# uthree/tinyvc

Hardware: AMD Instinct MI355X
Metric: audio-samples/sec (16 kHz) end-to-end VC (higher is better)
Workload: dtype f32 (fp32 in / out / accumulate; channel contractions as two-term fp16 splits on v_mfma_f32_32x32x16_f16: 22-bit significands, three part-products per fp32 product)

## Files before the change

### tinyvc_amd/csrc/knn.hip

```cpp
#include "knn_blob.h"
#include "knn_search.h"
#include "split_fp16.h"
#include "tvc_common.h"

namespace tvc {

constexpr int KNN_BLOCKS = 1024;

constexpr int QN_WAVES = 16;
static __global__ __launch_bounds__(QN_WAVES * 64) void query_normalize_kernel(const float* __restrict__ src, float* __restrict__ qn, int B, int Bsrc, int T,
                                                                     uint4* __restrict__ qh, int* __restrict__ cnt, int* __restrict__ flag,
                                                                     const KnnSegs segs, int* __restrict__ col2seg) {
    __shared__ float part[QN_WAVES][64];
    const int lane = threadIdx.x & 63, wave = threadIdx.x >> 6;
    const long ncols = (long)B * T;
    long n, nn;
    bool ok;
    int sg;
    if (qh) {
        const int tile = blockIdx.x >> 2;
        sg = seg_find<3>(segs, tile);
        const KnnSeg g = seg_get(segs, sg);
        const long loc = (long)(tile - g.u[3]) * 256 + (blockIdx.x & 3) * 64 + lane;
        ok = loc < g.ncols;
        n = g.col0 + loc;
        nn = ok ? n : g.col0 + g.ncols - 1;
    } else {
        n = blockIdx.x * 64L + lane;
        ok = n < ncols;
        nn = ok ? n : ncols - 1;
        sg = col2seg ? seg_find<4>(segs, (int)nn) : 0;
    }
    if (blockIdx.x == 0 && flag)
        for (int i = threadIdx.x; i < segs.n; i += QN_WAVES * 64) flag[i] = 0;
    if (wave == 0 && ok && cnt) cnt[n] = 0;
    if (wave == 0 && ok && col2seg) col2seg[n] = sg;
    const int b = (int)(nn / T), t = (int)(nn - (long)b * T);
    const float* p = src + (long)(b % Bsrc) * KD * T + t;
    float* q = qn + (long)b * KD * T + t;
    constexpr int KW = KD / QN_WAVES;
    const int k0 = wave * KW;
    float x[KW];
#pragma unroll
    for (int i = 0; i < KW; ++i) x[i] = p[(long)(k0 + i) * T];
    float s = 0.f;
#pragma unroll
    for (int i = 0; i < KW; ++i) s = fmaf(x[i], x[i], s);
    part[wave][lane] = s;
    __syncthreads();
    float ss = part[0][lane];
#pragma unroll
    for (int w = 1; w < QN_WAVES; ++w) ss += part[w][lane];
    const float den = sqrtf(ss) + 1e-6f;
    uint4* qhp = qh ? qh + (blockIdx.x >> 2) * (long)(STEPS * 2 * 256) + (blockIdx.x & 3) * 64 + lane : nullptr;
#pragma unroll
    for (int i = 0; i < KW; i += 8) {
        const int k = k0 + i;
        float v[8];
#pragma unroll
        for (int j = 0; j < 8; ++j) v[j] = ok ? x[i + j] / den : 0.f;
        if (ok) {
#pragma unroll
            for (int j = 0; j < 8; ++j) q[(long)(k + j) * T] = v[j];
        }
        if (qh) {
            unsigned o[4];
#pragma unroll
            for (int j = 0; j < 4; ++j) {
                const __half2 h = __floats2half2_rn(v[2 * j], v[2 * j + 1]);
                o[j] = (unsigned)__half_as_ushort(__low2half(h)) | ((unsigned)__half_as_ushort(__high2half(h)) << 16);
            }
            qhp[(long)(k >> 3) * 256] = make_uint4(o[0], o[1], o[2], o[3]);
        }
    }
}

typedef __bf16 bf16x8 __attribute__((ext_vector_type(8)));
typedef __bf16 bf16x2 __attribute__((ext_vector_type(2)));
__device__ __forceinline__ void split8_bf3(const float (&v)[8], uint4& p1, uint4& p2, uint4& p3) {
    unsigned o1[4], o2[4], o3[4];
#pragma unroll
    for (int j = 0; j < 4; ++j) {
        f32x2 a = {v[2 * j], v[2 * j + 1]};
        bf16x2 h1 = __builtin_convertvector(a, bf16x2);
        f32x2 r = a - __builtin_convertvector(h1, f32x2);
        bf16x2 h2 = __builtin_convertvector(r, bf16x2);
        f32x2 r2 = r - __builtin_convertvector(h2, f32x2);
        bf16x2 h3 = __builtin_convertvector(r2, bf16x2);
        o1[j] = __builtin_bit_cast(unsigned, h1);
        o2[j] = __builtin_bit_cast(unsigned, h2);
        o3[j] = __builtin_bit_cast(unsigned, h3);
    }
    p1 = make_uint4(o1[0], o1[1], o1[2], o1[3]);
    p2 = make_uint4(o2[0], o2[1], o2[2], o2[3]);
    p3 = make_uint4(o3[0], o3[1], o3[2], o3[3]);
}
__device__ __forceinline__ void split8_half(const u32x4 h8, uint4& p1, uint4& p2) {
    const f16x8 hv = __builtin_bit_cast(f16x8, h8);
    unsigned o1[4], o2[4];
#pragma unroll
    for (int j = 0; j < 4; ++j) {
        f32x2 a = {(float)hv[2 * j], (float)hv[2 * j + 1]};
        bf16x2 h1 = __builtin_convertvector(a, bf16x2);
        f32x2 r = a - __builtin_convertvector(h1, f32x2);
        bf16x2 h2 = __builtin_convertvector(r, bf16x2);
        o1[j] = __builtin_bit_cast(unsigned, h1);
        o2[j] = __builtin_bit_cast(unsigned, h2);
    }
    p1 = make_uint4(o1[0], o1[1], o1[2], o1[3]);
    p2 = make_uint4(o2[0], o2[1], o2[2], o2[3]);
}

constexpr int KNN_QT = 256;
constexpr int KNN_A_U4 = 12 * 64, KNN_X_U4 = 3 * 2 * KNN_QT;
template <bool F16>
__device__ __forceinline__ void knn_topk_body(const float* __restrict__ blob, long Npad, int N, const float* __restrict__ qn, int ncols, int col0, int cstride,
                                              int T, int unit, int nsplit, int tiles_per_split, float* __restrict__ cand_v, int* __restrict__ cand_i,
                                              uint4* smem) {
    constexpr int NP = F16 ? 2 : 3;
    constexpr int GP = F16 ? 4 : 12;
    uint4* As = smem;
    uint4* Xs = smem + 2 * KNN_A_U4;
    const uint4* img = F16 ? blob_img16(blob, KIND_F16, N, Npad) : blob_img3(blob, N);
    const float* inv = blob_inv(blob, KIND_F16, N, Npad);

    const int tid = threadIdx.x, lane = tid & 63, wave = tid >> 6;
    const int wm = wave >> 2, wn = wave & 3;
    const int l31 = lane & 31, lh = lane >> 5;
    const int split = unit % nsplit;
    const int qtile = unit / nsplit;
    const int n0 = qtile * KNN_QT;
    const int mtiles = (int)(Npad >> 7);
    const int mt_lo = split * tiles_per_split;
    const int mt_hi = min(mtiles, mt_lo + tiles_per_split);
    const int G = (mt_hi - mt_lo) * STEPS;

    const float* qp;
    int xdst;
    {
        const int g = tid >> 8, pos = tid & 255;
        int n = n0 + pos;
        n = col0 + (n < ncols ? n : ncols - 1);
        const int b = n / T, t = n - b * T;
        qp = qn + ((long)b * KD + 8 * g) * T + t;
        xdst = g * KNN_QT + pos;
    }
    const bool a2 = !F16 && wave < 4;
    const bool a1 = !F16 || wave < 4;
    float xr[8];
    u32x4 ar[2];
    auto gload = [&](int g) __attribute__((always_inline)) {
        const int mt = mt_lo + g / STEPS, st = g - (g / STEPS) * STEPS;
        const uint4* src = img + ((long)mt * STEPS + st) * (GP * 64) + lane;
        if (a1) ar[0] = *reinterpret_cast<const u32x4*>(src + wave * 64);
        if (a2) ar[1] = *reinterpret_cast<const u32x4*>(src + (wave + 8) * 64);
#pragma unroll
        for (int j = 0; j < 8; ++j) xr[j] = qp[(long)(st * 16 + j) * T];
    };
    auto lstore = [&](int buf) __attribute__((always_inline)) {
        uint4* ab = As + buf * KNN_A_U4;
        if (F16) {
            if (a1) {
                uint4 p1, p2;
                split8_half(ar[0], p1, p2);
                ab[(wave * 2) * 64 + lane] = p1;
                ab[(wave * 2 + 1) * 64 + lane] = p2;
            }
        } else {
            *reinterpret_cast<u32x4*>(ab + wave * 64 + lane) = ar[0];
            if (a2) *reinterpret_cast<u32x4*>(ab + (wave + 8) * 64 + lane) = ar[1];
        }
        uint4 p1, p2, p3;
        split8_bf3(xr, p1, p2, p3);
        uint4* xb = Xs + buf * KNN_X_U4;
        xb[xdst] = p1;
        xb[2 * KNN_QT + xdst] = p2;
        xb[4 * KNN_QT + xdst] = p3;
    };

    Top4 top[2];
    top[0].init();
    top[1].init();
    f32x16 acc[2][2];
#pragma unroll
    for (int i = 0; i < 2; ++i)
#pragma unroll
        for (int j = 0; j < 2; ++j)
#pragma unroll
            for (int r = 0; r < 16; ++r) acc[i][j][r] = 0.f;

    if (G > 0) {
        gload(0);
        lstore(0);
        if (G > 1) gload(1);
        slab_barrier();
    }
    for (int g = 0; g < G; ++g) {
        const int cur = g & 1;
        if (g + 1 < G) {
            lstore(cur ^ 1);
            if (g + 2 < G) gload(g + 2);
        }
        const uint4* as = As + cur * KNN_A_U4 + wm * (2 * NP * 64) + lane;
        const uint4* xs = Xs + cur * KNN_X_U4 + lh * KNN_QT + wn * 64 + l31;
        bf16x8 af[2][NP], bf[2][3];
#pragma unroll
        for (int j = 0; j < 2; ++j)
#pragma unroll
            for (int p = 0; p < 3; ++p) bf[j][p] = __builtin_bit_cast(bf16x8, xs[p * 2 * KNN_QT + j * 32]);
#pragma unroll
        for (int i = 0; i < 2; ++i)
#pragma unroll
            for (int p = 0; p < NP; ++p) af[i][p] = __builtin_bit_cast(bf16x8, as[(i * NP + p) * 64]);
        constexpr int NQ = F16 ? 5 : 6;
        constexpr int PA3[6] = {2, 1, 0, 1, 0, 0}, PB3[6] = {0, 1, 2, 0, 1, 0};
        constexpr int PA2[5] = {1, 0, 1, 0, 0}, PB2[5] = {1, 2, 0, 1, 0};
#pragma unroll
        for (int q = 0; q < NQ; ++q)
#pragma unroll
            for (int i = 0; i < 2; ++i)
#pragma unroll
                for (int j = 0; j < 2; ++j)
                    acc[i][j] = __builtin_amdgcn_mfma_f32_32x32x16_bf16(af[i][F16 ? PA2[q < 5 ? q : 0] : PA3[q]], bf[j][F16 ? PB2[q < 5 ? q : 0] : PB3[q]],
                                                                        acc[i][j], 0, 0, 0);
        const int st = g - (g / STEPS) * STEPS;
        if (st == STEPS - 1) {
            const int m0 = (mt_lo + g / STEPS) * 128;
#pragma unroll
            for (int i = 0; i < 2; ++i)
#pragma unroll
                for (int r = 0; r < 16; ++r) {
                    const int row = m0 + (wm * 2 + i) * 32 + (r & 3) + 8 * (r >> 2) + 4 * lh;
                    if (row < N) {
                        const float sc = F16 ? inv[row] : 1.f;
#pragma unroll
                        for (int j = 0; j < 2; ++j) top[j].insert(nan_max(F16 ? acc[i][j][r] * sc : acc[i][j][r]), row);
                    }
#pragma unroll
                    for (int j = 0; j < 2; ++j) acc[i][j][r] = 0.f;
                }
        }
        slab_barrier();
    }

    float (*mv)[16] = reinterpret_cast<float (*)[16]>(smem);
    int (*mi)[16] = reinterpret_cast<int (*)[16]>(reinterpret_cast<float*>(smem) + KNN_QT * 16);
#pragma unroll
    for (int j = 0; j < 2; ++j) {
        const int q = wn * 64 + j * 32 + l31;
        const int slot = (wm * 2 + lh) * 4;
#pragma unroll
        for (int e = 0; e < 4; ++e) {
            mv[q][slot + e] = top[j].v[e];
            mi[q][slot + e] = top[j].i[e];
        }
    }
    __syncthreads();
    if (tid < KNN_QT) {
        Top4 t4;
        t4.init();
        for (int e = 0; e < 16; ++e) t4.insert(mv[tid][e], mi[tid][e]);
        int n = n0 + tid;
        if (n < ncols) {
            long o = ((long)split * cstride + col0 + n) * 4;
#pragma unroll
            for (int e = 0; e < 4; ++e) {
                cand_v[o + e] = t4.v[e];
                cand_i[o + e] = t4.i[e];
            }
        }
    }
}

static __global__ __launch_bounds__(512) void knn_topk_split_kernel(const KnnSegs segs, const float* __restrict__ qn, int cstride, int T,
                                                                    float* __restrict__ cand_v, int* __restrict__ cand_i,
                                                                    const int* __restrict__ flags) {
    __shared__ __attribute__((aligned(16))) uint4 smem[2 * (KNN_A_U4 + KNN_X_U4)];
    const int si = seg_find<2>(segs, blockIdx.x);
    const KnnSeg g = seg_get(segs, si);
    if (g.two && flags[si] == 0) return;
    const int kind = blob_kind(g.blob);
    const int unit = blockIdx.x - g.u[2];
    if (kind == KIND_F16) knn_topk_body<true>(g.blob, blob_npad(g.N), g.N, qn, g.ncols, g.col0, cstride, T, unit, g.nsE, g.tpsE, cand_v, cand_i, smem);
    else knn_topk_body<false>(g.blob, blob_npad(g.N), g.N, qn, g.ncols, g.col0, cstride, T, unit, g.nsE, g.tpsE, cand_v, cand_i, smem);
}

constexpr int C_QT = 256, C_MT = 256, C_K = 64, C_STEPS = KD / C_K;
constexpr int C_A_U4 = 4 * 8 * 64, C_X_U4 = 4 * 2 * C_QT;
constexpr int C_LDS = 2 * (C_A_U4 + C_X_U4) * 16;
constexpr int C_CAP = 256;
constexpr float C_EPS = 1.25e-3f;
constexpr int KNN_COARSE_MIN = 4096;

struct Top4V {
    float v[4];
    __device__ __forceinline__ void init() { v[0] = v[1] = v[2] = v[3] = -INFINITY; }
    __device__ __forceinline__ void insert(float x) {
        if (!(x > v[3])) return;
        if (x > v[0]) { v[3] = v[2]; v[2] = v[1]; v[1] = v[0]; v[0] = x; }
        else if (x > v[1]) { v[3] = v[2]; v[2] = v[1]; v[1] = x; }
        else if (x > v[2]) { v[3] = v[2]; v[2] = x; }
        else v[3] = x;
    }
};

template <bool F16, int MODE>
static __device__ __forceinline__ void knn_coarse_body(const float* __restrict__ blob, long Npad, int N, const uint4* __restrict__ qh,
                                                       int ncols, int cstride, int unit, int nsplit, int tiles_per_split, int t2_cover,
                                                       float* __restrict__ c4v, int ns_sample,
                                                       int* __restrict__ cnt, int* __restrict__ cand, float* __restrict__ candv,
                                                       int* __restrict__ overflow) {
    extern __shared__ __attribute__((aligned(16))) uint4 csmem[];
    uint4* As = csmem;
    uint4* Xs = csmem + 2 * C_A_U4;
    const int kind = F16 ? KIND_F16 : KIND_F32;
    const uint4* img = blob_img16(blob, kind, N, Npad);
    const float* inv = blob_inv(blob, kind, N, Npad);

    const int tid = threadIdx.x, lane = tid & 63, wave = tid >> 6;
    const int wm = wave >> 2, wn = wave & 3;
    const int l31 = lane & 31, lh = lane >> 5;
    const int split = unit % nsplit;
    const int qtile = unit / nsplit;
    const int n0 = qtile * C_QT;
    const int mtiles = (int)(Npad >> 7);
    const int t_lo = split * tiles_per_split;
    const int t_hi = min(t2_cover, t_lo + tiles_per_split);
    const int G = (t_hi - t_lo) * C_STEPS;

    const uint4* xsrc = qh + (long)qtile * (STEPS * 2 * 256) + (tid & 511);
    u32x4 ar[4], xr[4];
    auto gload = [&](int g) __attribute__((always_inline)) {
        const int t2 = t_lo + g / C_STEPS, st = g - (g / C_STEPS) * C_STEPS;
#pragma unroll
        for (int i = 0; i < 4; ++i) {
            const int piece = wave + 8 * i, k16 = piece >> 3, mt8 = piece & 7;
            int t128 = 2 * t2 + (mt8 >> 2);
            t128 = t128 < mtiles ? t128 : mtiles - 1;
            ar[i] = *reinterpret_cast<const u32x4*>(img + (((long)t128 * STEPS + 4 * st + k16) * 4 + (mt8 & 3)) * 64 + lane);
            xr[i] = *reinterpret_cast<const u32x4*>(xsrc + (long)(4 * st + i) * 512);
        }
    };
    auto lstore = [&](int buf) __attribute__((always_inline)) {
#pragma unroll
        for (int i = 0; i < 4; ++i) {
            *reinterpret_cast<u32x4*>(As + buf * C_A_U4 + tid + 512 * i) = ar[i];
            *reinterpret_cast<u32x4*>(Xs + buf * C_X_U4 + tid + 512 * i) = xr[i];
        }
    };

    Top4V top[2];
    top[0].init();
    top[1].init();
    float th[2] = {INFINITY, INFINITY};
    if (MODE == 1) {
#pragma unroll
        for (int j = 0; j < 2; ++j) {
            const int n = n0 + wn * 64 + j * 32 + l31;
            if (n < ncols) {
                Top4V t4;
                t4.init();
                for (int sp = 0; sp < ns_sample; ++sp) {
                    const float4 v4 = *reinterpret_cast<const float4*>(c4v + ((long)sp * cstride + n) * 4);
                    t4.insert(v4.x);
                    t4.insert(v4.y);
                    t4.insert(v4.z);
                    t4.insert(v4.w);
// ... 64 lines not shown
                            const int row = m0 + (wm * 4 + i) * 32 + (r & 3) + 8 * (r >> 2) + 4 * lh;
                            if (whole || row < N) {
                                const float a = acc[i][j][r];
                                if (MODE == 0) {
                                    if (!F16) {
                                        top[j].insert(nan_max(a));
                                    } else if (!(fmaxf(a, 0.f) * imx <= top[j].v[3])) {
                                        top[j].insert(nan_max(a * inv[row]));
                                    }
                                } else {
                                    bool hit;
                                    float cv = a;
                                    if (!F16) hit = !(a < th[j]);
                                    else {
                                        hit = a != a || (fmaxf(a, 0.f) * imx >= th[j]);
                                        if (hit) {
                                            cv = a * inv[row];
                                            hit = a != a || cv >= th[j];
                                        }
                                    }
                                    hit = hit && th[j] != INFINITY;
                                    if (hit) {
                                        const int n = n0 + wn * 64 + j * 32 + l31;
                                        const int pos = atomicAdd(&cnt[n], 1);
                                        if (pos < C_CAP) {
                                            cand[(long)n * C_CAP + pos] = row;
                                            candv[(long)n * C_CAP + pos] = cv;
                                        } else *overflow = 1;
                                    }
                                }
                            }
                        }
                    }
#pragma unroll
                    for (int r = 0; r < 16; ++r) acc[i][j][r] = 0.f;
                }
        }
        slab_barrier();
    }
    if (MODE == 1) return;

    float (*mv)[16] = reinterpret_cast<float (*)[16]>(csmem);
#pragma unroll
    for (int j = 0; j < 2; ++j) {
        const int q = wn * 64 + j * 32 + l31;
        const int slot = (wm * 2 + lh) * 4;
#pragma unroll
        for (int e = 0; e < 4; ++e) mv[q][slot + e] = top[j].v[e];
    }
    __syncthreads();
    if (tid < C_QT) {
        Top4V t4;
        t4.init();
        for (int e = 0; e < 16; ++e) t4.insert(mv[tid][e]);
        const int n = n0 + tid;
        if (n < ncols) {
            const long o = ((long)split * cstride + n) * 4;
#pragma unroll
            for (int e = 0; e < 4; ++e) c4v[o + e] = t4.v[e];
        }
    }
}

template <int MODE>
static __global__ __launch_bounds__(512) void knn_coarse_kernel(const KnnSegs segs, const uint4* __restrict__ qh, int cstride,
                                                                float* __restrict__ c4v, int* __restrict__ cnt, int* __restrict__ cand,
                                                                float* __restrict__ candv, int* __restrict__ flags) {
    const int si = seg_find<MODE>(segs, blockIdx.x);
    const KnnSeg g = seg_get(segs, si);
    const int unit = blockIdx.x - g.u[MODE];
    const int nsplit = MODE ? g.nsB : g.nsA, tps = MODE ? g.tpsB : g.tpsA, cover = MODE ? g.t2 : g.sample;
    const uint4* q = qh + (long)g.u[3] * (STEPS * 2 * 256);
    float* c4 = c4v + (long)g.col0 * 4;
    int* ct = cnt + g.col0;
    int* cd = cand + (long)g.col0 * C_CAP;
    float* cdv = candv + (long)g.col0 * C_CAP;
    if (blob_kind(g.blob) == KIND_F16)
        knn_coarse_body<true, MODE>(g.blob, blob_npad(g.N), g.N, q, g.ncols, cstride, unit, nsplit, tps, cover, c4, g.nsA, ct, cd, cdv, flags + si);
    else
        knn_coarse_body<false, MODE>(g.blob, blob_npad(g.N), g.N, q, g.ncols, cstride, unit, nsplit, tps, cover, c4, g.nsA, ct, cd, cdv, flags + si);
}

static __global__ __launch_bounds__(256) void knn_rescore_kernel(const KnnSegs segs, const int* __restrict__ col2seg, const float* __restrict__ qn,
                                                                 int ncols, int T, const int* __restrict__ cnt, const int* __restrict__ cand,
                                                                 const float* __restrict__ candv, float* __restrict__ rv, int* __restrict__ ri) {
    constexpr int RG = 4;
    const int lane = threadIdx.x & 63;
    const int n = blockIdx.x * 4 + (threadIdx.x >> 6);
    if (n >= ncols) return;
    const KnnSeg g = seg_get(segs, col2seg ? __builtin_amdgcn_readfirstlane(col2seg[n]) : 0);
    if (!g.two) return;
    const float* __restrict__ blob = g.blob;
    const int N = g.N;
    const long Npad = blob_npad(g.N);
    const int kind = blob_kind(blob);
    const float* inv = blob_inv(blob, kind, N, Npad);
    const int b = n / T, t = n - b * T;
    const float* qp = qn + (long)b * KD * T + t;
    int rowl[C_CAP / 64];
    float cvl[C_CAP / 64];
#pragma unroll
    for (int c = 0; c < C_CAP / 64; ++c) {
        rowl[c] = cand[(long)n * C_CAP + 64 * c + lane];
        cvl[c] = candv[(long)n * C_CAP + 64 * c + lane];
    }
    const int nc = min(cnt[n], C_CAP);
    Top4 t4;
    t4.init();
    float th2;
    {
        float rk[C_CAP / 64];
#pragma unroll
        for (int c = 0; c < C_CAP / 64; ++c) {
            if (!(64 * c + lane < nc)) {
                cvl[c] = -INFINITY;
                rowl[c] = 0;
            }
            rk[c] = cvl[c] == cvl[c] ? cvl[c] : -INFINITY;
        }
        float wm = -INFINITY;
#pragma unroll
        for (int round = 0; round < 4; ++round) {
            float lm = rk[0];
#pragma unroll
            for (int c = 1; c < C_CAP / 64; ++c) lm = fmaxf(lm, rk[c]);
            wm = lm;
#pragma unroll
            for (int o = 32; o > 0; o >>= 1) wm = fmaxf(wm, __shfl_xor(wm, o));
            const unsigned long long who = __builtin_amdgcn_ballot_w64(lm == wm);
            if (lane == __builtin_ctzll(who)) {
                bool done = false;
#pragma unroll
                for (int c = 0; c < C_CAP / 64; ++c)
                    if (!done && rk[c] == wm) {
                        rk[c] = -INFINITY;
                        done = true;
                    }
            }
        }
        th2 = wm - 2.f * C_EPS;
    }
    static_assert(C_CAP == 256, "four 64-entry chunks");
    if (kind == KIND_F16) {
        const uint4* img = blob_img16(blob, kind, N, Npad);
        float qs[2][8];
#pragma unroll
        for (int h = 0; h < 2; ++h)
#pragma unroll
            for (int j = 0; j < 8; ++j) {
                const int seg = lane + 64 * h;
                qs[h][j] = seg < 96 ? qp[(long)(8 * seg + j) * T] : 0.f;
            }
        for (int base = 0, ch = 0; base < nc; base += 64, ++ch) {
            const int mine = ch == 0 ? rowl[0] : (ch == 1 ? rowl[1] : (ch == 2 ? rowl[2] : rowl[3]));
            const float cvv = ch == 0 ? cvl[0] : (ch == 1 ? cvl[1] : (ch == 2 ? cvl[2] : cvl[3]));
            unsigned long long mask = __builtin_amdgcn_ballot_w64(base + lane < nc && !(cvv < th2));
            while (mask) {
                int row[RG];
                bool live[RG];
                float d[RG], iv[RG];
                u32x4 w[RG][2];
                int pos = 0;
#pragma unroll
                for (int g = 0; g < RG; ++g) {
                    live[g] = mask != 0ull;
                    if (live[g]) {
                        pos = __builtin_ctzll(mask);
                        mask &= mask - 1;
                    }
                    row[g] = __shfl(mine, pos);
                    const long rbase = ((long)(row[g] >> 7) * STEPS * 4 + ((row[g] & 127) >> 5)) * 64 + (row[g] & 31);
#pragma unroll
                    for (int h = 0; h < 2; ++h) {
                        const int seg = lane + 64 * h < 96 ? lane + 64 * h : 0;
                        w[g][h] = *reinterpret_cast<const u32x4*>(img + rbase + (long)(seg >> 1) * 256 + (seg & 1) * 32);
                    }
                    iv[g] = inv[row[g]];
                }
#pragma unroll
                for (int g = 0; g < RG; ++g) {
                    d[g] = 0.f;
#pragma unroll
                    for (int h = 0; h < 2; ++h) {
                        if (lane + 64 * h < 96) {
                            const f16x8 hv = __builtin_bit_cast(f16x8, w[g][h]);
#pragma unroll
                            for (int j = 0; j < 8; ++j) d[g] = fmaf(qs[h][j], (float)hv[j], d[g]);
                        }
                    }
                }
#pragma unroll
                for (int o = 32; o > 0; o >>= 1)
#pragma unroll
                    for (int g = 0; g < RG; ++g) d[g] += __shfl_xor(d[g], o);
#pragma unroll
                for (int g = 0; g < RG; ++g)
                    if (live[g]) t4.insert(nan_max(d[g] * iv[g]), row[g]);
            }
        }
    } else {
        float qv[12];
#pragma unroll
        for (int u = 0; u < 12; ++u) qv[u] = qp[(long)(lane + 64 * u) * T];
        const float* rows = blob_rows(blob);
        for (int base = 0, ch = 0; base < nc; base += 64, ++ch) {
            const int mine = ch == 0 ? rowl[0] : (ch == 1 ? rowl[1] : (ch == 2 ? rowl[2] : rowl[3]));
            const float cvv = ch == 0 ? cvl[0] : (ch == 1 ? cvl[1] : (ch == 2 ? cvl[2] : cvl[3]));
            unsigned long long mask = __builtin_amdgcn_ballot_w64(base + lane < nc && !(cvv < th2));
            while (mask) {
                int row[RG];
                bool live[RG];
                float d[RG], iv[RG], xv[RG][12];
                int pos = 0;
#pragma unroll
                for (int g = 0; g < RG; ++g) {
                    live[g] = mask != 0ull;
                    if (live[g]) {
                        pos = __builtin_ctzll(mask);
                        mask &= mask - 1;
                    }
                    row[g] = __shfl(mine, pos);
                    const float* rp = rows + (long)row[g] * KD + lane;
#pragma unroll
                    for (int u = 0; u < 12; ++u) xv[g][u] = rp[64 * u];
                    iv[g] = inv[row[g]];
                }
#pragma unroll
                for (int g = 0; g < RG; ++g) {
                    d[g] = 0.f;
#pragma unroll
                    for (int u = 0; u < 12; ++u) d[g] = fmaf(qv[u], xv[g][u], d[g]);
                }
#pragma unroll
                for (int o = 32; o > 0; o >>= 1)
#pragma unroll
                    for (int g = 0; g < RG; ++g) d[g] += __shfl_xor(d[g], o);
#pragma unroll
                for (int g = 0; g < RG; ++g)
                    if (live[g]) t4.insert(nan_max(d[g] * iv[g]), row[g]);
            }
        }
    }
    if (nc < 4) {
#pragma unroll
        for (int e = 0; e < 4; ++e) {
            t4.v[e] = INFINITY;
            t4.i[e] = e;
        }
    }
    if (lane == 0) {
#pragma unroll
        for (int e = 0; e < 4; ++e) {
            rv[(long)n * 4 + e] = t4.v[e];
            ri[(long)n * 4 + e] = t4.i[e];
        }
    }
}

static void split_plan(int blocks, int qtiles, int cover, int* ns, int* tps) {
    int n = (blocks + qtiles - 1) / qtiles;
    if (n > cover) n = cover;
    if (n < 1) n = 1;
    *tps = (cover + n - 1) / n;
    *ns = (cover + *tps - 1) / *tps;
}

int knn_call_plan(tvc_ctx* ctx, const KnnSegIn* in, int nin, int ncols, KnnCall* c) {
    static_assert(KNN_QT == C_QT, "one query tiling for both searches");
    c->ncols = ncols;
    for (int i = 0; i < nin; ++i) {
        if (in[i].N > 0x7fffff00L) return fail(ctx, TVC_ERR_ARG, "index too large");
        if (in[i].ncols <= 0) continue;
        if (!c->seg.empty() && c->seg.back().blob == in[i].blob && c->seg.back().col0 + c->seg.back().ncols == in[i].col0) {
            c->seg.back().ncols += in[i].ncols;
            continue;
        }
        KnnSeg g{};
        g.blob = in[i].blob;
        g.N = (int)in[i].N;
        g.col0 = in[i].col0;
        g.ncols = in[i].ncols;
        c->seg.push_back(g);
    }
    if (c->seg.empty()) return fail(ctx, TVC_ERR_ARG, "knn: no query columns");
    for (auto& g : c->seg) c->cq += (g.ncols + C_QT - 1) / C_QT;
    int mt_max = 1;
    int tile = 0;
    for (auto& g : c->seg) {
        const long Npad = blob_npad(g.N);
        const int mtiles = (int)(Npad / 128);
        const int qt = (g.ncols + C_QT - 1) / C_QT;
        mt_max = mtiles > mt_max ? mtiles : mt_max;
        g.two = g.N >= KNN_COARSE_MIN;
        g.t2 = (int)((Npad + C_MT - 1) / C_MT);
        g.sample = g.t2 / 8 < 5 ? 5 : g.t2 / 8;
        if (g.sample > g.t2) g.sample = g.t2;
        split_plan(768, c->cq, g.sample, &g.nsA, &g.tpsA);
        split_plan(768, c->cq, g.t2, &g.nsB, &g.tpsB);
        split_plan(KNN_BLOCKS, c->cq, mtiles, &g.nsE, &g.tpsE);
        g.u[0] = c->units[0];
        g.u[1] = c->units[1];
        g.u[2] = c->units[2];
        g.u[3] = tile;
        if (g.two) {
            c->units[0] += qt * g.nsA;
            c->units[1] += qt * g.nsB;
            c->two = true;
        }
        c->units[2] += qt * g.nsE;
        tile += qt;
    }
    if (c->seg.size() == 1) c->ns_cv = c->seg[0].nsE;
    else {
        const int cq_min = (ncols + C_QT - 1) / C_QT;
        c->ns_cv = (KNN_BLOCKS + cq_min - 1) / cq_min;
        c->ns_cv = c->ns_cv < mt_max ? c->ns_cv : mt_max;
    }
    return 0;
}

template <int MODE>
static int coarse_launch(tvc_ctx* ctx, hipStream_t s, const KnnCall& c, const KnnLists& L, const uint4* qh, float* c4v, int* cnt, int* cand, float* candv) {
    TVC_CHECK(lds_optin<knn_coarse_kernel<MODE>>(ctx, C_LDS, "knn coarse"));
    hipLaunchKernelGGL((knn_coarse_kernel<MODE>), dim3((unsigned)c.units[MODE]), dim3(512), C_LDS, s, L.segs, qh, c.ncols, c4v, cnt, cand, candv, L.flag);
    return 0;
}

static int coarse_max_nsplit(int qtiles) { return (768 + qtiles - 1) / qtiles; }

int knn_candidates(tvc_ctx* ctx, hipStream_t s, Ws& ws, const float* src, const KnnCall& c, int B, int T, KnnLists* L, int Bsrc) {
    const int nseg = (int)c.seg.size();
    float* qn = ws.get<float>((size_t)B * KD * T);
    L->cv = ws.get<float>((size_t)c.ns_cv * c.ncols * 4);
    L->ci = ws.get<int>((size_t)c.ns_cv * c.ncols * 4);
    int* dtab = nseg > 1 ? ws.get<int>((size_t)nseg * sizeof(KnnSeg) / sizeof(int)) : nullptr;
    L->col2seg = nseg > 1 ? ws.get<int>((size_t)c.ncols) : nullptr;
    uint4* qh = nullptr;
    float* c4v = nullptr;
    int *cnt = nullptr, *cand = nullptr;
    float* candv = nullptr;
    if (c.two) {
        qh = ws.get<uint4>((size_t)c.cq * STEPS * 2 * 256);
        c4v = ws.get<float>((size_t)coarse_max_nsplit((c.ncols + C_QT - 1) / C_QT) * c.ncols * 4);
        cnt = ws.get<int>((size_t)c.ncols);
        cand = ws.get<int>((size_t)c.ncols * C_CAP);
        candv = ws.get<float>((size_t)c.ncols * C_CAP);
        L->rv = ws.get<float>((size_t)c.ncols * 4);
        L->ri = ws.get<int>((size_t)c.ncols * 4);
        L->flag = ws.get<int>((size_t)(nseg > 64 ? nseg : 64));
    }
    if (ws.dry) return 0;
    L->segs.n = nseg;
    L->segs.one = c.seg[0];
    L->segs.d = reinterpret_cast<const KnnSeg*>(dtab);
    if (dtab) {
        std::vector<int> words((size_t)nseg * sizeof(KnnSeg) / sizeof(int));
        std::memcpy(words.data(), c.seg.data(), words.size() * sizeof(int));
        TVC_CHECK(upload_ints(ctx, s, words, dtab));
    }
    const int nblk = c.two ? c.cq * 4 : (c.ncols + 63) / 64;
    hipLaunchKernelGGL(query_normalize_kernel, dim3(nblk), dim3(QN_WAVES * 64), 0, s, src, qn, B, Bsrc > 0 ? Bsrc : B, T, qh, cnt, L->flag, L->segs, L->col2seg);
    if (c.two) {
        ProfScope ps(ctx, s, ws, "knn.coarse+rescore");
        TVC_CHECK((coarse_launch<0>(ctx, s, c, *L, qh, c4v, cnt, cand, candv)));
        TVC_CHECK((coarse_launch<1>(ctx, s, c, *L, qh, c4v, cnt, cand, candv)));
        hipLaunchKernelGGL(knn_rescore_kernel, dim3((c.ncols + 3) / 4), dim3(256), 0, s, L->segs, (const int*)L->col2seg, qn, c.ncols, T, cnt, cand, candv, L->rv, L->ri);
    }
    ProfScope ps(ctx, s, ws, "knn.exact");
    hipLaunchKernelGGL(knn_topk_split_kernel, dim3((unsigned)c.units[2]), dim3(512), 0, s, L->segs, qn, c.ncols, T, L->cv, L->ci, (const int*)L->flag);
    return 0;
}

}
```

### tinyvc_amd/csrc/knn_gather.hip

```cpp
#include "knn_blob.h"
#include "knn_search.h"
#include "tvc_common.h"

namespace tvc {

__device__ __forceinline__ Top4 merge_lists(const float* __restrict__ cv, const int* __restrict__ ci, int nsplit, long stride, long col) {
    Top4 t4;
    t4.init();
    for (int s = 0; s < nsplit; ++s) {
        const long o = (s * stride + col) * 4;
        for (int e = 0; e < 4; ++e) t4.insert(cv[o + e], ci[o + e]);
    }
    return t4;
}
__device__ __forceinline__ void merged_top4(const KnnSeg& g, int si, const int* __restrict__ flags, const float* __restrict__ cand_v,
                                            const int* __restrict__ cand_i, const float* __restrict__ rv, const int* __restrict__ ri, long stride,
                                            long col, bool live, int64_t* __restrict__ idx_out, int* sel) {
    const bool rescored = g.two && flags[si] == 0;
    Top4 t4;
    t4.init();
    if (live) {
        t4 = merge_lists(rescored ? rv : cand_v, rescored ? ri : cand_i, rescored ? 1 : g.nsE, stride, col);
        for (int e = 0; e < 4; ++e) t4.i[e] = (unsigned)t4.i[e] < (unsigned)g.N ? t4.i[e] : 0;
        if (idx_out)
            for (int e = 0; e < 4; ++e) idx_out[col * 4 + e] = (int64_t)t4.i[e];
    }
    for (int e = 0; e < 4; ++e) sel[e] = live ? t4.i[e] : 0;
}
struct RowSrc { const float* blob; int kind, N; };
template <class Src>
__device__ __forceinline__ void gather4x3(float (&r)[4][3][4], int q0, Src src, const int (*sel)[4], int k) {
#pragma unroll
    for (int qq = 0; qq < 4; ++qq) {
        const int q = q0 + 4 * qq;
        const RowSrc b = src(q);
        const long Npad = blob_npad(b.N);
#pragma unroll
        for (int u = 0; u < 3; ++u)
#pragma unroll
            for (int e = 0; e < 4; ++e) r[qq][u][e] = blob_row_value(b.blob, b.kind, b.N, Npad, sel[q][e], k + 64 * u);
    }
}
__device__ __forceinline__ float mean4(float r0, float r1, float r2, float r3) {
    return __fadd_rn(__fadd_rn(__fadd_rn(r0, r1), r2), r3) * 0.25f;
}
__device__ __forceinline__ void store_tile_along_t(const float (&tile)[32][193], float* __restrict__ out, int n0, int ncols, int T, int kc) {
    for (int kk = threadIdx.x >> 5; kk < 192; kk += 8) {
        const int q = threadIdx.x & 31;
        const int n = n0 + q;
        if (n < ncols) {
            const int b = n / T, t = n - b * T;
            out[((long)b * KD + kc + kk) * T + t] = tile[q][kk];
        }
    }
}

struct AlphaIn {
    const float* alpha;
    const float* src;
    const int* col2b;
    const int* rowmap;
};
__device__ __forceinline__ float alpha_of_column(const AlphaIn& al, int nc, int T) { return al.alpha[al.col2b ? al.rowmap[al.col2b[nc]] : nc / T]; }
struct ShareIn {
    const float* share;
    const float* src;
};
__device__ __forceinline__ float alpha_of_column(const ShareIn& sh, int nc, int) { return sh.share[nc]; }
template <class AI>
__device__ __forceinline__ void store_tile_along_t_alpha(const float (&tile)[32][193], float* __restrict__ out, const AI& al, float a, int n0,
                                                         int ncols, int T, int kc) {
    const float* __restrict__ src = al.src;
    const float keep = __fsub_rn(1.f, a);
    for (int kk = threadIdx.x >> 5; kk < 192; kk += 8) {
        const int q = threadIdx.x & 31;
        const int n = n0 + q;
        if (n < ncols) {
            const int b = n / T, t = n - b * T;
            const long o = ((long)b * KD + kc + kk) * T + t;
            out[o] = __fadd_rn(__fmul_rn(tile[q][kk], keep), __fmul_rn(src[o], a));
        }
    }
}

template <bool MULTI, class... A>
static __global__ __launch_bounds__(256) void knn_merge_gather_kernel(const float* __restrict__ cand_v, const int* __restrict__ cand_i,
                                                                      const KnnSegs segs, const int* __restrict__ col2seg, int ncols, int T,
                                                                      float* __restrict__ out, int64_t* __restrict__ idx_out,
                                                                      const float* __restrict__ rv, const int* __restrict__ ri,
                                                                      const int* __restrict__ flags, const A... al) {
    constexpr bool ALPHA = sizeof...(A) > 0;
    __shared__ int sel[32][4];
    __shared__ float tile[32][193];
    __shared__ const float* sblob[32];
    __shared__ int skind[32], sN[32];
    const int tid = threadIdx.x;
    const int n0 = blockIdx.x * 32;
    float a = 0.f;
    if constexpr (ALPHA) {
        const int n = n0 + (tid & 31);
        a = alpha_of_column(al..., n < ncols ? n : ncols - 1, T);
    }
    if (tid < 32) {
        const int n = n0 + tid;
        const int nc = n < ncols ? n : ncols - 1;
        const int si = MULTI ? col2seg[nc] : 0;
        const KnnSeg g = seg_get(segs, si);
        merged_top4(g, si, flags, cand_v, cand_i, rv, ri, ncols, n, n < ncols, idx_out, sel[tid]);
        if (MULTI) {
            sblob[tid] = g.blob;
            skind[tid] = blob_kind(g.blob);
            sN[tid] = g.N;
        }
    }
    __syncthreads();
    const int lane = tid & 63, wave = tid >> 6;
    const RowSrc one{segs.one.blob, MULTI ? 0 : blob_kind(segs.one.blob), segs.one.N};
    for (int kc = 0; kc < KD; kc += 192) {
        for (int q0 = wave; q0 < 32; q0 += 16) {
            float r[4][3][4];
            if (MULTI) gather4x3(r, q0, [&](int q) { return RowSrc{sblob[q], skind[q], sN[q]}; }, sel, kc + lane);
            else gather4x3(r, q0, [&](int) { return one; }, sel, kc + lane);
#pragma unroll
            for (int qq = 0; qq < 4; ++qq)
#pragma unroll
                for (int u = 0; u < 3; ++u) tile[q0 + 4 * qq][lane + 64 * u] = mean4(r[qq][u][0], r[qq][u][1], r[qq][u][2], r[qq][u][3]);
        }
        __syncthreads();
        if constexpr (ALPHA) store_tile_along_t_alpha(tile, out, al..., a, n0, ncols, T, kc);
        else store_tile_along_t(tile, out, n0, ncols, T, kc);
        __syncthreads();
    }
}

constexpr int BLEND_MAX = TVC_BLEND_MAX;
template <class... A>
static __global__ __launch_bounds__(256) void knn_merge_blend_gather_kernel(const float* __restrict__ cand_v, const int* __restrict__ cand_i,
                                                                            const KnnSegs segs, const int* __restrict__ col2seg, int ncols, int T,
                                                                            int M, const float* __restrict__ weights, const int* __restrict__ col2b,
                                                                            const int* __restrict__ rowmap, float* __restrict__ out,
                                                                            int64_t* __restrict__ idx_out, const float* __restrict__ rv,
                                                                            const int* __restrict__ ri, const int* __restrict__ flags, const A... al) {
    constexpr bool ALPHA = sizeof...(A) > 0;
    __shared__ int sel[BLEND_MAX][32][4];
    __shared__ float tile[32][193];
    __shared__ const float* sblob[BLEND_MAX][32];
    __shared__ int skind[BLEND_MAX][32], sN[BLEND_MAX][32];
    __shared__ float sw[BLEND_MAX][32];
    const int tid = threadIdx.x;
    const int n0 = blockIdx.x * 32;
    float a = 0.f;
    if constexpr (ALPHA) {
        const int n = n0 + (tid & 31);
        a = alpha_of_column(al..., n < ncols ? n : ncols - 1, T);
    }
    if (tid < 32 * M) {
        const int m = tid >> 5, q = tid & 31;
        const int n = n0 + q;
        const bool live = n < ncols;
        const int nc = live ? n : ncols - 1;
        const long vcols = (long)M * ncols;
        const long vc = (long)m * ncols + nc;
        const int si = col2seg ? col2seg[vc] : 0;
        const KnnSeg g = seg_get(segs, si);
        merged_top4(g, si, flags, cand_v, cand_i, rv, ri, vcols, vc, live, idx_out, sel[m][q]);
        sblob[m][q] = g.blob;
        skind[m][q] = blob_kind(g.blob);
        sN[m][q] = g.N;
        const int row = col2b ? rowmap[col2b[nc]] : nc / T;
        sw[m][q] = weights[(long)row * M + m];
    }
    __syncthreads();
    const int lane = tid & 63, wave = tid >> 6;
    for (int kc = 0; kc < KD; kc += 192) {
        for (int q0 = wave; q0 < 32; q0 += 16) {
            float acc[4][3];
#pragma unroll 1
            for (int m = 0; m < M; ++m) {
                float r[4][3][4];
                gather4x3(r, q0, [&](int q) { return RowSrc{sblob[m][q], skind[m][q], sN[m][q]}; }, sel[m], kc + lane);
#pragma unroll
                for (int qq = 0; qq < 4; ++qq) {
                    const float w = sw[m][q0 + 4 * qq];
#pragma unroll
                    for (int u = 0; u < 3; ++u) {
                        const float term = __fmul_rn(w, mean4(r[qq][u][0], r[qq][u][1], r[qq][u][2], r[qq][u][3]));
                        acc[qq][u] = m == 0 ? term : __fadd_rn(acc[qq][u], term);
                    }
                }
            }
#pragma unroll
            for (int qq = 0; qq < 4; ++qq)
#pragma unroll
                for (int u = 0; u < 3; ++u) tile[q0 + 4 * qq][lane + 64 * u] = acc[qq][u];
        }
        __syncthreads();
        if constexpr (ALPHA) store_tile_along_t_alpha(tile, out, al..., a, n0, ncols, T, kc);
        else store_tile_along_t(tile, out, n0, ncols, T, kc);
        __syncthreads();
    }
}

static __global__ __launch_bounds__(256) void alpha_bound_kernel(const float* __restrict__ alpha, const int* __restrict__ row,
                                                                 const float* __restrict__ idx_bound, int stride, const float* __restrict__ srcmax,
                                                                 float* __restrict__ out, int n) {
    const int i = blockIdx.x * 256 + threadIdx.x;
    if (i >= n) return;
    const float a = alpha[row ? row[i] : i];
    out[i] = __fadd_rn(__fmul_rn(fabsf(__fsub_rn(1.f, a)), idx_bound[(long)i * stride]), __fmul_rn(fabsf(a), srcmax[i]));
}
__device__ __forceinline__ float share_of_frame(float a, float p, float w) { return __fadd_rn(a, __fmul_rn(__fsub_rn(1.f, a), __fmul_rn(p, w))); }
static __global__ __launch_bounds__(256) void protect_bound_kernel(const float* __restrict__ alpha, const float* __restrict__ protect,
                                                                   const int* __restrict__ row, const float* __restrict__ idx_bound, int stride,
                                                                   const float* __restrict__ srcmax, float* __restrict__ out, int n) {
    const int i = blockIdx.x * 256 + threadIdx.x;
// ... 118 lines not shown
static __global__ __launch_bounds__(256) void knn_merge_kernel(const float* __restrict__ cand_v, const int* __restrict__ cand_i, int nsplit, int ncols,
                                                               float* __restrict__ sims_out, int64_t* __restrict__ idx_out,
                                                               const float* __restrict__ rv, const int* __restrict__ ri, const int* __restrict__ flag) {
    const int n = blockIdx.x * 256 + threadIdx.x;
    if (n >= ncols) return;
    if (flag && *flag == 0) {
        cand_v = rv;
        cand_i = ri;
        nsplit = 1;
    }
    const Top4 t4 = merge_lists(cand_v, cand_i, nsplit, ncols, n);
    for (int e = 0; e < 4; ++e) {
        sims_out[(long)n * 4 + e] = t4.v[e];
        idx_out[(long)n * 4 + e] = (int64_t)t4.i[e];
    }
}
static __global__ __launch_bounds__(192) void knn_slot_gather_kernel(const float* __restrict__ blob, const int64_t* __restrict__ idx, long nslots,
                                                                     long N, long Npad, float* __restrict__ slots) {
    const long sl = blockIdx.x;
    if (sl >= nslots) return;
    const int kind = blob_kind(blob);
    const int64_t i = idx[sl];
    float4 v = make_float4(0.f, 0.f, 0.f, 0.f);
    if (i >= 0 && i < N) {
        const int k = 4 * threadIdx.x;
        v = make_float4(blob_row_value(blob, kind, N, Npad, i, k), blob_row_value(blob, kind, N, Npad, i, k + 1),
                        blob_row_value(blob, kind, N, Npad, i, k + 2), blob_row_value(blob, kind, N, Npad, i, k + 3));
    }
    reinterpret_cast<float4*>(slots + sl * KD)[threadIdx.x] = v;
}
static __global__ __launch_bounds__(256) void knn_finish_kernel(const float* __restrict__ slots, int ncols, int T, float* __restrict__ out) {
    __shared__ float tile[32][193];
    const int tid = threadIdx.x, lane = tid & 63, wave = tid >> 6;
    const int n0 = blockIdx.x * 32;
    for (int kc = 0; kc < KD; kc += 192) {
        for (int q = wave; q < 32; q += 4) {
            const int n = n0 + q < ncols ? n0 + q : ncols - 1;
            const float* r0 = slots + ((long)n * 4) * KD + kc;
#pragma unroll
            for (int u = 0; u < 3; ++u) {
                const int k = lane + 64 * u;
                tile[q][k] = mean4(r0[k], r0[KD + k], r0[2 * KD + k], r0[3 * KD + k]);
            }
        }
        __syncthreads();
        store_tile_along_t(tile, out, n0, ncols, T, kc);
        __syncthreads();
    }
}

int run_knn_topk(tvc_ctx* ctx, hipStream_t s, Ws& ws, const float* src, const float* prepared, int64_t N,
                 float* sims_out, int64_t* idx_out, int B, int T) {
    const KnnSegIn one{prepared, N, 0, B * T};
    KnnCall c;
    TVC_CHECK(knn_call_plan(ctx, &one, 1, B * T, &c));
    KnnLists L;
    TVC_CHECK(knn_candidates(ctx, s, ws, src, c, B, T, &L));
    if (ws.dry) return 0;
    hipLaunchKernelGGL(knn_merge_kernel, dim3((c.ncols + 255) / 256), dim3(256), 0, s, L.cv, L.ci, c.seg[0].nsE, c.ncols, sims_out, idx_out, L.rv, L.ri, L.flag);
    return launch_check(ctx, "knn_topk");
}

int run_knn_slots(tvc_ctx* ctx, hipStream_t s, const float* prepared, int64_t N, const int64_t* idx, float* slots, int64_t nslots) {
    hipLaunchKernelGGL(knn_slot_gather_kernel, dim3((unsigned)nslots), dim3(192), 0, s, prepared, idx, (long)nslots, (long)N, blob_npad(N), slots);
    return launch_check(ctx, "knn_slots");
}

int run_knn_finish(tvc_ctx* ctx, hipStream_t s, const float* slots, float* out, int B, int T) {
    const int ncols = B * T;
    hipLaunchKernelGGL(knn_finish_kernel, dim3((ncols + 31) / 32), dim3(256), 0, s, slots, ncols, T, out);
    return launch_check(ctx, "knn_finish");
}

int run_knn_segs(tvc_ctx* ctx, hipStream_t s, Ws& ws, const float* src, const KnnSegIn* in, int nin, float* out, int64_t* idx_out, int B, int T,
                 const float* alpha, const float* share) {
    KnnCall c;
    TVC_CHECK(knn_call_plan(ctx, in, nin, B * T, &c));
    KnnLists L;
    TVC_CHECK(knn_candidates(ctx, s, ws, src, c, B, T, &L));
    if (ws.dry) return 0;
    if (share) {
        const ShareIn sh{share, src};
        const auto skernel = L.col2seg ? knn_merge_gather_kernel<true, ShareIn> : knn_merge_gather_kernel<false, ShareIn>;
        hipLaunchKernelGGL(skernel, dim3((c.ncols + 31) / 32), dim3(256), 0, s, L.cv, L.ci, L.segs, (const int*)L.col2seg, c.ncols, T, out, idx_out, L.rv, L.ri,
                           (const int*)L.flag, sh);
        return launch_check(ctx, "knn_match_protect");
    }
    if (alpha) {
        const RagHost* h = ctx->rag;
        const AlphaIn al{alpha, src, h ? (const int*)h->d_col2b : (const int*)nullptr, h ? (const int*)h->d_row : (const int*)nullptr};
        const auto akernel = L.col2seg ? knn_merge_gather_kernel<true, AlphaIn> : knn_merge_gather_kernel<false, AlphaIn>;
        hipLaunchKernelGGL(akernel, dim3((c.ncols + 31) / 32), dim3(256), 0, s, L.cv, L.ci, L.segs, (const int*)L.col2seg, c.ncols, T, out, idx_out, L.rv, L.ri,
                           (const int*)L.flag, al);
        return launch_check(ctx, "knn_match_alpha");
    }
    const auto kernel = L.col2seg ? knn_merge_gather_kernel<true> : knn_merge_gather_kernel<false>;
    hipLaunchKernelGGL(kernel, dim3((c.ncols + 31) / 32), dim3(256), 0, s, L.cv, L.ci, L.segs, (const int*)L.col2seg, c.ncols, T, out, idx_out, L.rv, L.ri,
                       (const int*)L.flag);
    return launch_check(ctx, "knn_match");
}

int run_knn_blend(tvc_ctx* ctx, hipStream_t s, Ws& ws, const float* src, const KnnSegIn* in, int nin, int M, const float* weights, float* out,
                  int64_t* idx_out, int B, int T, const float* alpha, const float* share) {
    KnnCall c;
    TVC_CHECK(knn_call_plan(ctx, in, nin, M * B * T, &c));
    KnnLists L;
    TVC_CHECK(knn_candidates(ctx, s, ws, src, c, M * B, T, &L, B));
    if (ws.dry) return 0;
    const RagHost* h = ctx->rag;
    if (share) {
        const ShareIn sh{share, src};
        hipLaunchKernelGGL(knn_merge_blend_gather_kernel<ShareIn>, dim3((B * T + 31) / 32), dim3(256), 0, s, L.cv, L.ci, L.segs, (const int*)L.col2seg, B * T, T, M,
                           weights, h ? (const int*)h->d_col2b : (const int*)nullptr, h ? (const int*)h->d_row : (const int*)nullptr, out, idx_out, L.rv, L.ri,
                           (const int*)L.flag, sh);
        return launch_check(ctx, "knn_match_blend_protect");
    }
    if (alpha) {
        const int* col2b = h ? (const int*)h->d_col2b : nullptr;
        const int* rowmap = h ? (const int*)h->d_row : nullptr;
        const AlphaIn al{alpha, src, col2b, rowmap};
        hipLaunchKernelGGL(knn_merge_blend_gather_kernel<AlphaIn>, dim3((B * T + 31) / 32), dim3(256), 0, s, L.cv, L.ci, L.segs, (const int*)L.col2seg, B * T, T, M,
                           weights, col2b, rowmap, out, idx_out, L.rv, L.ri, (const int*)L.flag, al);
        return launch_check(ctx, "knn_match_blend_alpha");
    }
    hipLaunchKernelGGL(knn_merge_blend_gather_kernel<>, dim3((B * T + 31) / 32), dim3(256), 0, s, L.cv, L.ci, L.segs, (const int*)L.col2seg, B * T, T, M, weights,
                       h ? (const int*)h->d_col2b : (const int*)nullptr, h ? (const int*)h->d_row : (const int*)nullptr, out, idx_out, L.rv, L.ri,
                       (const int*)L.flag);
    return launch_check(ctx, "knn_match_blend");
}

int run_knn(tvc_ctx* ctx, hipStream_t s, Ws& ws, const float* src, const float* prepared, int64_t N,
            float* out, int64_t* idx_out, int B, int T) {
    const KnnSegIn one{prepared, N, 0, B * T};
    return run_knn_segs(ctx, s, ws, src, &one, 1, out, idx_out, B, T);
}

}
```

Measured before the change: 712.9 million.

## Store normalized queries query-major and split merge-gather across feature chunks

When the coarse path is active, the query normalize kernel now transposes through shared memory and writes normalized queries in query-major layout. The exact top-k and rescore kernels read them with contiguous float4 loads instead of strided per-channel loads. Separately, the merge-gather kernel now spreads the 192-wide feature chunks across a second grid dimension with 8 waves, instead of looping over chunks inside one block. This adds parallelism, but each chunk block recomputes the top-4 merge. The added transpose scratch in shared memory also raises LDS use, which may lower occupancy of the normalize kernel.

After: 719.6 million, median of 6. Within noise of the previous version (+0.9%).

```diff
diff --git a/tinyvc_amd/csrc/knn.hip b/tinyvc_amd/csrc/knn.hip
--- a/tinyvc_amd/csrc/knn.hip
+++ b/tinyvc_amd/csrc/knn.hip
@@ -12,6 +12,7 @@
                                                                      uint4* __restrict__ qh, int* __restrict__ cnt, int* __restrict__ flag,
                                                                      const KnnSegs segs, int* __restrict__ col2seg) {
     __shared__ float part[QN_WAVES][64];
+    __shared__ float tr[QN_WAVES][64][17];
     const int lane = threadIdx.x & 63, wave = threadIdx.x >> 6;
     const long ncols = (long)B * T;
     long n, nn;
@@ -53,13 +54,29 @@
     for (int w = 1; w < QN_WAVES; ++w) ss += part[w][lane];
     const float den = sqrtf(ss) + 1e-6f;
     uint4* qhp = qh ? qh + (blockIdx.x >> 2) * (long)(STEPS * 2 * 256) + (blockIdx.x & 3) * 64 + lane : nullptr;
+    const int nlive = __popcll(__builtin_amdgcn_ballot_w64(ok));
+    float* qmp = qn + (n - lane) * KD + k0 + 4 * (lane & 3);
 #pragma unroll
     for (int i = 0; i < KW; i += 8) {
         const int k = k0 + i;
         float v[8];
 #pragma unroll
         for (int j = 0; j < 8; ++j) v[j] = ok ? x[i + j] / den : 0.f;
-        if (ok) {
+        if (qh) {
+#pragma unroll
+            for (int j = 0; j < 8; ++j) tr[wave][lane][(i & 8) + j] = v[j];
+            if (i & 8) {
+                __builtin_amdgcn_wave_barrier();
+#pragma unroll
+                for (int r = 0; r < 4; ++r) {
+                    const int c = (lane >> 2) + 16 * r;
+                    const float* tp = &tr[wave][c][4 * (lane & 3)];
+                    const float4 o = make_float4(tp[0], tp[1], tp[2], tp[3]);
+                    if (c < nlive) *reinterpret_cast<float4*>(qmp + (long)c * KD + (i - 8)) = o;
+                }
+                __builtin_amdgcn_wave_barrier();
+            }
+        } else if (ok) {
 #pragma unroll
             for (int j = 0; j < 8; ++j) q[(long)(k + j) * T] = v[j];
         }
@@ -114,8 +131,8 @@
 constexpr int KNN_QT = 256;
 constexpr int KNN_A_U4 = 12 * 64, KNN_X_U4 = 3 * 2 * KNN_QT;
 template <bool F16>
-__device__ __forceinline__ void knn_topk_body(const float* __restrict__ blob, long Npad, int N, const float* __restrict__ qn, int ncols, int col0, int cstride,
-                                              int T, int unit, int nsplit, int tiles_per_split, float* __restrict__ cand_v, int* __restrict__ cand_i,
+__device__ __forceinline__ void knn_topk_body(const float* __restrict__ blob, long Npad, int N, const float* __restrict__ qn, bool qmajor, int ncols, int col0,
+                                              int cstride, int T, int unit, int nsplit, int tiles_per_split, float* __restrict__ cand_v, int* __restrict__ cand_i,
                                               uint4* smem) {
     constexpr int NP = F16 ? 2 : 3;
     constexpr int GP = F16 ? 4 : 12;
@@ -142,7 +159,7 @@
         int n = n0 + pos;
         n = col0 + (n < ncols ? n : ncols - 1);
         const int b = n / T, t = n - b * T;
-        qp = qn + ((long)b * KD + 8 * g) * T + t;
+        qp = qmajor ? qn + (long)n * KD + 8 * g : qn + ((long)b * KD + 8 * g) * T + t;
         xdst = g * KNN_QT + pos;
     }
     const bool a2 = !F16 && wave < 4;
@@ -154,8 +171,14 @@
         const uint4* src = img + ((long)mt * STEPS + st) * (GP * 64) + lane;
         if (a1) ar[0] = *reinterpret_cast<const u32x4*>(src + wave * 64);
         if (a2) ar[1] = *reinterpret_cast<const u32x4*>(src + (wave + 8) * 64);
-#pragma unroll
-        for (int j = 0; j < 8; ++j) xr[j] = qp[(long)(st * 16 + j) * T];
+        if (qmajor) {
+            const float4* q4 = reinterpret_cast<const float4*>(qp + st * 16);
+            const float4 lo = q4[0], hi = q4[1];
+            xr[0] = lo.x, xr[1] = lo.y, xr[2] = lo.z, xr[3] = lo.w, xr[4] = hi.x, xr[5] = hi.y, xr[6] = hi.z, xr[7] = hi.w;
+        } else {
+#pragma unroll
+            for (int j = 0; j < 8; ++j) xr[j] = qp[(long)(st * 16 + j) * T];
+        }
     };
     auto lstore = [&](int buf) __attribute__((always_inline)) {
         uint4* ab = As + buf * KNN_A_U4;
@@ -281,8 +304,8 @@
     if (g.two && flags[si] == 0) return;
     const int kind = blob_kind(g.blob);
     const int unit = blockIdx.x - g.u[2];
-    if (kind == KIND_F16) knn_topk_body<true>(g.blob, blob_npad(g.N), g.N, qn, g.ncols, g.col0, cstride, T, unit, g.nsE, g.tpsE, cand_v, cand_i, smem);
-    else knn_topk_body<false>(g.blob, blob_npad(g.N), g.N, qn, g.ncols, g.col0, cstride, T, unit, g.nsE, g.tpsE, cand_v, cand_i, smem);
+    if (kind == KIND_F16) knn_topk_body<true>(g.blob, blob_npad(g.N), g.N, qn, flags != nullptr, g.ncols, g.col0, cstride, T, unit, g.nsE, g.tpsE, cand_v, cand_i, smem);
+    else knn_topk_body<false>(g.blob, blob_npad(g.N), g.N, qn, flags != nullptr, g.ncols, g.col0, cstride, T, unit, g.nsE, g.tpsE, cand_v, cand_i, smem);
 }
 
 constexpr int C_QT = 256, C_MT = 256, C_K = 64, C_STEPS = KD / C_K;
@@ -513,7 +536,7 @@
 }
 
 static __global__ __launch_bounds__(256) void knn_rescore_kernel(const KnnSegs segs, const int* __restrict__ col2seg, const float* __restrict__ qn,
-                                                                 int ncols, int T, const int* __restrict__ cnt, const int* __restrict__ cand,
+                                                                 int ncols, const int* __restrict__ cnt, const int* __restrict__ cand,
                                                                  const float* __restrict__ candv, float* __restrict__ rv, int* __restrict__ ri) {
     constexpr int RG = 4;
     const int lane = threadIdx.x & 63;
@@ -526,8 +549,7 @@
     const long Npad = blob_npad(g.N);
     const int kind = blob_kind(blob);
     const float* inv = blob_inv(blob, kind, N, Npad);
-    const int b = n / T, t = n - b * T;
-    const float* qp = qn + (long)b * KD * T + t;
+    const float* qp = qn + (long)n * KD;
     int rowl[C_CAP / 64];
     float cvl[C_CAP / 64];
 #pragma unroll
@@ -576,12 +598,14 @@
         const uint4* img = blob_img16(blob, kind, N, Npad);
         float qs[2][8];
 #pragma unroll
-        for (int h = 0; h < 2; ++h)
-#pragma unroll
-            for (int j = 0; j < 8; ++j) {
-                const int seg = lane + 64 * h;
-                qs[h][j] = seg < 96 ? qp[(long)(8 * seg + j) * T] : 0.f;
-            }
+        for (int h = 0; h < 2; ++h) {
+            const int seg = lane + 64 * h;
+            const float4* q4 = reinterpret_cast<const float4*>(qp + 8 * (seg < 96 ? seg : 0));
+            const float4 lo = q4[0], hi = q4[1];
+            const float got[8] = {lo.x, lo.y, lo.z, lo.w, hi.x, hi.y, hi.z, hi.w};
+#pragma unroll
+            for (int j = 0; j < 8; ++j) qs[h][j] = seg < 96 ? got[j] : 0.f;
+        }
         for (int base = 0, ch = 0; base < nc; base += 64, ++ch) {
             const int mine = ch == 0 ? rowl[0] : (ch == 1 ? rowl[1] : (ch == 2 ? rowl[2] : rowl[3]));
             const float cvv = ch == 0 ? cvl[0] : (ch == 1 ? cvl[1] : (ch == 2 ? cvl[2] : cvl[3]));
@@ -632,7 +656,7 @@
     } else {
         float qv[12];
 #pragma unroll
-        for (int u = 0; u < 12; ++u) qv[u] = qp[(long)(lane + 64 * u) * T];
+        for (int u = 0; u < 12; ++u) qv[u] = qp[lane + 64 * u];
         const float* rows = blob_rows(blob);
         for (int base = 0, ch = 0; base < nc; base += 64, ++ch) {
             const int mine = ch == 0 ? rowl[0] : (ch == 1 ? rowl[1] : (ch == 2 ? rowl[2] : rowl[3]));
@@ -795,7 +819,7 @@
         ProfScope ps(ctx, s, ws, "knn.coarse+rescore");
         TVC_CHECK((coarse_launch<0>(ctx, s, c, *L, qh, c4v, cnt, cand, candv)));
         TVC_CHECK((coarse_launch<1>(ctx, s, c, *L, qh, c4v, cnt, cand, candv)));
-        hipLaunchKernelGGL(knn_rescore_kernel, dim3((c.ncols + 3) / 4), dim3(256), 0, s, L->segs, (const int*)L->col2seg, qn, c.ncols, T, cnt, cand, candv, L->rv, L->ri);
+        hipLaunchKernelGGL(knn_rescore_kernel, dim3((c.ncols + 3) / 4), dim3(256), 0, s, L->segs, (const int*)L->col2seg, (const float*)qn, c.ncols, cnt, cand, candv, L->rv, L->ri);
     }
     ProfScope ps(ctx, s, ws, "knn.exact");
     hipLaunchKernelGGL(knn_topk_split_kernel, dim3((unsigned)c.units[2]), dim3(512), 0, s, L->segs, qn, c.ncols, T, L->cv, L->ci, (const int*)L->flag);
diff --git a/tinyvc_amd/csrc/knn_gather.hip b/tinyvc_amd/csrc/knn_gather.hip
--- a/tinyvc_amd/csrc/knn_gather.hip
+++ b/tinyvc_amd/csrc/knn_gather.hip
@@ -45,7 +45,7 @@
     return __fadd_rn(__fadd_rn(__fadd_rn(r0, r1), r2), r3) * 0.25f;
 }
 __device__ __forceinline__ void store_tile_along_t(const float (&tile)[32][193], float* __restrict__ out, int n0, int ncols, int T, int kc) {
-    for (int kk = threadIdx.x >> 5; kk < 192; kk += 8) {
+    for (int kk = threadIdx.x >> 5; kk < 192; kk += blockDim.x >> 5) {
         const int q = threadIdx.x & 31;
         const int n = n0 + q;
         if (n < ncols) {
@@ -72,7 +72,7 @@
                                                          int ncols, int T, int kc) {
     const float* __restrict__ src = al.src;
     const float keep = __fsub_rn(1.f, a);
-    for (int kk = threadIdx.x >> 5; kk < 192; kk += 8) {
+    for (int kk = threadIdx.x >> 5; kk < 192; kk += blockDim.x >> 5) {
         const int q = threadIdx.x & 31;
         const int n = n0 + q;
         if (n < ncols) {
@@ -83,8 +83,9 @@
     }
 }
 
+constexpr int MG_WAVES = 8;
 template <bool MULTI, class... A>
-static __global__ __launch_bounds__(256) void knn_merge_gather_kernel(const float* __restrict__ cand_v, const int* __restrict__ cand_i,
+static __global__ __launch_bounds__(MG_WAVES * 64) void knn_merge_gather_kernel(const float* __restrict__ cand_v, const int* __restrict__ cand_i,
                                                                       const KnnSegs segs, const int* __restrict__ col2seg, int ncols, int T,
                                                                       float* __restrict__ out, int64_t* __restrict__ idx_out,
                                                                       const float* __restrict__ rv, const int* __restrict__ ri,
@@ -106,7 +107,7 @@
         const int nc = n < ncols ? n : ncols - 1;
         const int si = MULTI ? col2seg[nc] : 0;
         const KnnSeg g = seg_get(segs, si);
-        merged_top4(g, si, flags, cand_v, cand_i, rv, ri, ncols, n, n < ncols, idx_out, sel[tid]);
+        merged_top4(g, si, flags, cand_v, cand_i, rv, ri, ncols, n, n < ncols, blockIdx.y == 0 ? idx_out : nullptr, sel[tid]);
         if (MULTI) {
             sblob[tid] = g.blob;
             skind[tid] = blob_kind(g.blob);
@@ -116,21 +117,19 @@
     __syncthreads();
     const int lane = tid & 63, wave = tid >> 6;
     const RowSrc one{segs.one.blob, MULTI ? 0 : blob_kind(segs.one.blob), segs.one.N};
-    for (int kc = 0; kc < KD; kc += 192) {
-        for (int q0 = wave; q0 < 32; q0 += 16) {
-            float r[4][3][4];
-            if (MULTI) gather4x3(r, q0, [&](int q) { return RowSrc{sblob[q], skind[q], sN[q]}; }, sel, kc + lane);
-            else gather4x3(r, q0, [&](int) { return one; }, sel, kc + lane);
-#pragma unroll
-            for (int qq = 0; qq < 4; ++qq)
-#pragma unroll
-                for (int u = 0; u < 3; ++u) tile[q0 + 4 * qq][lane + 64 * u] = mean4(r[qq][u][0], r[qq][u][1], r[qq][u][2], r[qq][u][3]);
-        }
-        __syncthreads();
-        if constexpr (ALPHA) store_tile_along_t_alpha(tile, out, al..., a, n0, ncols, T, kc);
-        else store_tile_along_t(tile, out, n0, ncols, T, kc);
-        __syncthreads();
-    }
+    static_assert(MG_WAVES == 8, "two groups of four waves: queries 0..15 and 16..31");
+    const int kc = blockIdx.y * 192;
+    const int q0 = (wave & 3) + 16 * (wave >> 2);
+    float r[4][3][4];
+    if (MULTI) gather4x3(r, q0, [&](int q) { return RowSrc{sblob[q], skind[q], sN[q]}; }, sel, kc + lane);
+    else gather4x3(r, q0, [&](int) { return one; }, sel, kc + lane);
+#pragma unroll
+    for (int qq = 0; qq < 4; ++qq)
+#pragma unroll
+        for (int u = 0; u < 3; ++u) tile[q0 + 4 * qq][lane + 64 * u] = mean4(r[qq][u][0], r[qq][u][1], r[qq][u][2], r[qq][u][3]);
+    __syncthreads();
+    if constexpr (ALPHA) store_tile_along_t_alpha(tile, out, al..., a, n0, ncols, T, kc);
+    else store_tile_along_t(tile, out, n0, ncols, T, kc);
 }
 
 constexpr int BLEND_MAX = TVC_BLEND_MAX;
@@ -415,7 +414,7 @@
     if (share) {
         const ShareIn sh{share, src};
         const auto skernel = L.col2seg ? knn_merge_gather_kernel<true, ShareIn> : knn_merge_gather_kernel<false, ShareIn>;
-        hipLaunchKernelGGL(skernel, dim3((c.ncols + 31) / 32), dim3(256), 0, s, L.cv, L.ci, L.segs, (const int*)L.col2seg, c.ncols, T, out, idx_out, L.rv, L.ri,
+        hipLaunchKernelGGL(skernel, dim3((c.ncols + 31) / 32, KD / 192), dim3(MG_WAVES * 64), 0, s, L.cv, L.ci, L.segs, (const int*)L.col2seg, c.ncols, T, out, idx_out, L.rv, L.ri,
                            (const int*)L.flag, sh);
         return launch_check(ctx, "knn_match_protect");
     }
@@ -423,12 +422,12 @@
         const RagHost* h = ctx->rag;
         const AlphaIn al{alpha, src, h ? (const int*)h->d_col2b : (const int*)nullptr, h ? (const int*)h->d_row : (const int*)nullptr};
         const auto akernel = L.col2seg ? knn_merge_gather_kernel<true, AlphaIn> : knn_merge_gather_kernel<false, AlphaIn>;
-        hipLaunchKernelGGL(akernel, dim3((c.ncols + 31) / 32), dim3(256), 0, s, L.cv, L.ci, L.segs, (const int*)L.col2seg, c.ncols, T, out, idx_out, L.rv, L.ri,
+        hipLaunchKernelGGL(akernel, dim3((c.ncols + 31) / 32, KD / 192), dim3(MG_WAVES * 64), 0, s, L.cv, L.ci, L.segs, (const int*)L.col2seg, c.ncols, T, out, idx_out, L.rv, L.ri,
                            (const int*)L.flag, al);
         return launch_check(ctx, "knn_match_alpha");
     }
     const auto kernel = L.col2seg ? knn_merge_gather_kernel<true> : knn_merge_gather_kernel<false>;
-    hipLaunchKernelGGL(kernel, dim3((c.ncols + 31) / 32), dim3(256), 0, s, L.cv, L.ci, L.segs, (const int*)L.col2seg, c.ncols, T, out, idx_out, L.rv, L.ri,
+    hipLaunchKernelGGL(kernel, dim3((c.ncols + 31) / 32, KD / 192), dim3(MG_WAVES * 64), 0, s, L.cv, L.ci, L.segs, (const int*)L.col2seg, c.ncols, T, out, idx_out, L.rv, L.ri,
                        (const int*)L.flag);
     return launch_check(ctx, "knn_match");
 }
```
